# rock-slam/slam-pose_estimation

Measured on AMD Instinct MI355X. Metric: UKF predict+update filter-cycles/s, PoseWithVelocity filters, higher is better.
Workload: dtype f64

## Files before the change

slam-pose_estimation_amd/csrc/ukf_kernel16.hpp:

```cpp
#pragma once

#include <type_traits>

#include "ukf_kernel.hpp"

namespace ukfb {

template <int CTRL> UKFB_DEV float dpp_mov(float v) {
    return __builtin_bit_cast(float, __builtin_amdgcn_update_dpp(0, __builtin_bit_cast(int, v), CTRL, 0xF, 0xF, true));
}
template <int CTRL> UKFB_DEV double dpp_mov(double v) {
    const unsigned long long b = __builtin_bit_cast(unsigned long long, v);
    const int lo = __builtin_amdgcn_update_dpp(0, int(unsigned(b)), CTRL, 0xF, 0xF, true);
    const int hi = __builtin_amdgcn_update_dpp(0, int(unsigned(b >> 32)), CTRL, 0xF, 0xF, true);
    return __builtin_bit_cast(double, (unsigned long long)(unsigned)lo | ((unsigned long long)(unsigned)hi << 32));
}
template <int C> UKFB_DEV float row_bcast(float v) { return dpp_mov<0x150 + C>(v); }
template <int C> UKFB_DEV double row_bcast(double v) { return __builtin_amdgcn_update_dpp(0.0, v, 0x150 + C, 0xF, 0xF, true); }
template <int C> UKFB_DEV void fmac_bcast(float& acc, float src, float m) {
    asm volatile("v_fmac_f32_dpp %0, %1, %2 row_newbcast:%3 row_mask:0xf bank_mask:0xf" : "+v"(acc) : "v"(src), "v"(m), "n"(C));
}
template <int C> UKFB_DEV void fmac_bcast(double& acc, double src, double m) {
    asm volatile("v_fmac_f64_dpp %0, %1, %2 row_newbcast:%3 row_mask:0xf bank_mask:0xf" : "+v"(acc) : "v"(src), "v"(m), "n"(C));
}
// ... 107 lines not shown
};

constexpr float ISO_TOL_F32 = 1e-4f;
template <class T, class M> struct Layout16 {
    static constexpr int VEC = 16 / int(sizeof(T));
    static constexpr int D = M::D, S = M::S, N = 2 * D + 1, PK = D * (D + 1) / 2;
    static constexpr int LS = 14;
    static constexpr int al(int x) { return (x + VEC - 1) / VEC * VEC; }
    static constexpr int PKP = al(PK);
    static constexpr int NL = 6, ST = (D == 12) ? 6 : 7, TRIP = D + 1;
    static constexpr int LC = 0;
    static constexpr int TNL = (D * LS > N * ST) ? (D * LS - N * ST) : 0;
    static constexpr bool ORIENT64_TRIM = (M::MODEL == 1 && sizeof(T) == 8);
    static constexpr bool LAF_ROW_D = !(M::MODEL == 0 || ORIENT64_TRIM);
    static constexpr int alm(int x) { return (M::MODEL == 0 && sizeof(T) == 4) ? (x + 1) / 2 * 2 : al(x); }
    static constexpr int UEND = al(TNL + (N + 1) * ST);
    static constexpr int PKS = UEND;
    static constexpr int LAF = PKS + PKP;
    static constexpr int LAF_SZ = al((D + (LAF_ROW_D ? 1 : 0)) * ST);
    static constexpr int LAF_PAD = LAF_ROW_D ? 0 : (LAF_SZ - D * ST);
    static constexpr int MISC = LAF + LAF_SZ;
    static constexpr int MUS = MISC;
    static constexpr int ROT = MUS + alm(S);
    static constexpr int ZQ = ROT + alm(9);
    static constexpr int NSH = ZQ + 12;
    static constexpr bool SINK_IN_NSH = ORIENT64_TRIM;
    static constexpr int NSH_SINK = SINK_IN_NSH ? (NSH + 21) : (NSH + alm(21));
    static constexpr int DUM = SINK_IN_NSH ? NSH : (NSH + alm(21));
    static constexpr int PF_RAW = SINK_IN_NSH ? (NSH + alm(21)) : (DUM + alm(S));
    static_assert(!SINK_IN_NSH || (alm(21) > 21 && alm(21) >= S), "the sink fits the noise table, which has a spare slot");
    __host__ __device__ static constexpr int cv(int r, int c) { return PKS + r * (r + 1) / 2 + c; }
    static constexpr int PF = PF_RAW + (((PF_RAW * int(sizeof(T)) / 4) % 32 == 0) ? 2 * VEC : 0);
    static_assert(TNL + N * ST >= D * LS && D - NL <= ST && NL <= ST, "prediction tables");
    static_assert(PF % 2 == 0 && LS >= D && LS <= 16 && S <= 16 && D + 1 <= 16, "scratch layout");
};

template <class T, class M> constexpr int lds_bytes_per_filter16() { return Layout16<T, M>::PF * int(sizeof(T)); }

template <class T, class M, class TS = T> struct CovTab {
    using LY = Layout16<T, M>;
    static constexpr int D = M::D, NL = LY::NL, ST = LY::ST, TRIP = LY::TRIP, TR = MT<M>::TR, TC = MT<M>::TC;
    static constexpr int NAB = (D - NL) * (D - NL + 1) / 2, AEL = (NAB + 15) / 16;
    static constexpr int NRD = 8, NWR = 16, SZ = int(sizeof(T)), SZG = int(sizeof(TS));
    static constexpr int RD_PR = 0, RD_PC = 1, RD_WS = 2, RD_NZ = 4, RD_ANZ = 5;
    static constexpr int WR_TILE = 0, WR_AFF = TR * TC, WR_AFF_RD = TR * TC + AEL;
    static_assert(RD_ANZ + AEL <= NRD && WR_AFF_RD + AEL <= NWR, "covariance lane tables");
    struct Tabs {
        uint32_t rd[16][NRD];
        uint32_t wr[17][NWR];
    };
    static constexpr int tri_r(int e) {
        int r = 0;
        while ((r + 1) * (r + 2) / 2 <= e) ++r;
        return r;
    }
    static constexpr Tabs make() {
        Tabs t{};
        const uint32_t sink = uint32_t(LY::DUM * SZ);
        for (int l = 0; l < 16; ++l) {
            const int lw = (l < MT<M>::WORK_LANES) ? l : 0;
            const int R0 = int((MT<M>::TILE_R >> (4 * lw)) & 15ull), C0 = int((MT<M>::TILE_C >> (4 * lw)) & 15ull);
            const bool is_cross = R0 >= NL;
            const int half = is_cross ? 0 : (lw & 1);
            t.rd[l][RD_PR] = uint32_t((is_cross ? (LY::LAF + (R0 - NL)) : (LY::TNL + half * (TRIP * ST) + R0)) * SZ);
            t.rd[l][RD_PC] = uint32_t((LY::TNL + ((is_cross || half) ? (TRIP * ST) : 0) + C0) * SZ);
            if (SZ == 8) {
                t.rd[l][RD_WS] = 0u;
                t.rd[l][RD_WS + 1] = is_cross ? 0u : 0x3FF00000u;
            } else {
                t.rd[l][RD_WS] = is_cross ? 0u : 0x3F800000u;
            }
            const int rc0 = R0 < D ? R0 : D - 1, cc0 = C0 < D ? C0 : D - 1;
            t.rd[l][RD_NZ] = uint32_t((rc0 * D + cc0) * SZG);
            const bool writer = (l < MT<M>::WORK_LANES) && (is_cross || half == 0);
            for (int i2 = 0; i2 < TR; ++i2)
                for (int j2 = 0; j2 < TC; ++j2) {
                    const int r = R0 + i2, c = C0 + j2;
                    const bool w = writer && r < D && c <= r;
                    t.wr[l][WR_TILE + i2 * TC + j2] = w ? uint32_t(LY::cv(r, c) * SZ) : sink;
                }
            for (int k = 0; k < AEL; ++k) {
                const int e = l + 16 * k;
                const bool v = e < NAB;
                const int rr = v ? tri_r(e) : 0, cc = v ? (e - rr * (rr + 1) / 2) : 0;
                const int ar = NL + rr, ac = NL + cc;
                t.rd[l][RD_ANZ + k] = uint32_t((ar * D + ac) * SZG);
                t.wr[l][WR_AFF + k] = v ? uint32_t(LY::cv(ar, ac) * SZ) : sink;
                t.wr[l][WR_AFF_RD + k] = uint32_t(LY::cv(ar, ac) * SZ);
            }
        }
        for (int k = 0; k < NWR; ++k) t.wr[16][k] = sink;
        for (int k = 0; k < AEL; ++k) t.wr[16][WR_AFF_RD + k] = uint32_t(LY::cv(NL, NL) * SZ);
        return t;
    }
    static constexpr Tabs tabs = make();
};

template <class T, class M, class TS = T> struct OCovTab {
    using LY = Layout16<T, M>;
    static constexpr int D = M::D, NL = LY::NL, ST = LY::ST, TRIP = LY::TRIP, TR = MT<M>::TR, TC = MT<M>::TC;
    static constexpr int NAB = (D - NL) * (D - NL + 1) / 2, AEL = (NAB + 15) / 16, SZ = int(sizeof(T)), SZG = int(sizeof(TS));
    static constexpr int RD_PR = 0, RD_PC = 1, RD_FLAGS = 2, RD_NZ = 3, RD_ANZ = 4, NRD = 8;
    static constexpr int WR_TILE = 0, WR_AFF = TR * TC, WR_AFF_RD = TR * TC + AEL, NWR = 16;
    static_assert(AEL == 2 && TR * TC + 2 * AEL <= NWR && RD_ANZ + AEL <= NRD, "OrientationState lane tables");
    struct Tabs {
        uint16_t rd[16][NRD];
        uint16_t wr[17][NWR];
    };
    static constexpr int tri_r(int e) {
        int r = 0;
// ... 86 lines not shown
#endif
UKFB_DEV void keep(float& x) { asm volatile("" : "+v"(x)); }
UKFB_DEV void keep(double& x) { asm volatile("" : "+v"(x)); }

template <class T, int D, int LS, int KS = D, int PUB = KS> UKFB_DEV T chol16(T (&a)[D], T* Lc, int l, bool& ok) {
    static_assert(PUB <= KS && KS <= D, "chol16 column counts");
    bool good = true;
    const int lw = (l < D) ? l : (D - 1);
    static_for<0, KS>([&](auto kc) {
        constexpr int k = decltype(kc)::value;
        dpp_hazard_fence(a[k]);
        if constexpr (k >= PUB) {
            const T akk = row_bcast<k>(a[k]);
            good = good && (akk > T(0));
        }
        const T nt = -(a[k] * rcp_bcast<k>(a[k]));
        if constexpr (k + 1 < KS) {
            static_for<k + 1, KS>([&](auto cc) {
                constexpr int c = decltype(cc)::value;
                fmac_bcast<c>(a[c], a[k], nt);
            });
        }
    });
#pragma unroll
    for (int k = 0; k < PUB; ++k) Lc[k * LS + lw] = (l >= k) ? a[k] : T(0);
    wsync();
    const int lc = (l < PUB) ? l : (PUB - 1);
    const T pv = Lc[lc * LS + lc];
    constexpr unsigned long long NO_PIVOT = ((0xFFFFull << PUB) & 0xFFFFull) * 0x0001000100010001ull;
    ok = good && row_all(NO_PIVOT | lanes_gt(pv, T(0)));
    return fast_rsqrt(pv);
}

template <class T, int D> UKFB_DEV void load_row(const T* PKS, int l, T (&row)[D]) {
    const int lr = (l < D) ? l : (D - 1);
    const T* p = PKS + lr * (lr + 1) / 2;
#pragma unroll
    for (int j = 0; j < D; ++j) row[j] = p[j];
}

template <class T, int D, int LS> UKFB_DEV void load_column(const T* Lc, int l, T rs, T (&col)[D]) {
    const int lc = (l < D) ? l : (D - 1);
    const T w = (l < D) ? rs : T(0);
#pragma unroll
    for (int c = 0; c < D; ++c) col[c] = Lc[lc * LS + c] * w;
}

template <class T> UKFB_DEV void rot_minus(const T (&qx)[4], const T (&qy)[4], T (&r)[3]) {
    const T oc[4] = {-qy[0], -qy[1], -qy[2], qy[3]};
    T d[4];
    quat_mul(oc, qx, d);
    so3_log_fast(d, r);
}

template <class T> UKFB_DEV void rot_minus_n2(const T (&qxa)[4], const T (&qxb)[4], const T (&qy)[4], T nrm, T (&ra)[3], T (&rb)[3]) {
    const T oc[4] = {-qy[0], -qy[1], -qy[2], qy[3]};
    T da[4], db[4];
    quat_mul(oc, qxa, da);
    quat_mul(oc, qxb, db);
    if constexpr (sizeof(T) == 4) {
        so3_log_fast_n2(da, db, nrm, ra, rb);
    } else {
        so3_log_fast_n(da, nrm, ra);
        so3_log_fast_n(db, nrm, rb);
    }
}

template <class T> UKFB_DEV void rot_minus_n(const T (&qx)[4], const T (&qy)[4], T nrm, T (&r)[3]) {
    const T oc[4] = {-qy[0], -qy[1], -qy[2], qy[3]};
    T d[4];
    quat_mul(oc, qx, d);
// ... 50 lines not shown
template <class T, class M>
UKFB_DEV void sigma_pair(const T (&mu)[M::S], const T (&col)[M::D], T (&xp)[M::S], T (&xm)[M::S]) {
    constexpr int Q = MT<M>::Q, RT = MT<M>::RT, S = M::S;
#pragma unroll
    for (int s = 0; s < S; ++s) {
        if (s < Q) { xp[s] = mu[s] + col[s]; xm[s] = mu[s] - col[s]; }
        else if (s >= Q + 4) { xp[s] = mu[s] + col[s - 1]; xm[s] = mu[s] - col[s - 1]; }
    }
    const T q[4] = {mu[Q], mu[Q + 1], mu[Q + 2], mu[Q + 3]};
    const T v[3] = {col[RT], col[RT + 1], col[RT + 2]};
    T ep[4], rp[4], rm[4];
    so3_exp_fast(v, T(1), ep);
    quat_mul_pm(q, ep, rp, rm);
#pragma unroll
    for (int k = 0; k < 4; ++k) { xp[Q + k] = rp[k]; xm[Q + k] = rm[k]; }
}

template <class T, class M, class TS>
UKFB_DEV T process_noise_entry16(const TS* Rn, const TS* Racc, const T* ROT, const ProcIn<T>& pin, int r, int c) {
    constexpr int D = M::D;
    T vacc = T(0);
    if (M::MODEL == 0) {
        vacc = T(Racc[r * D + c]);
    }
    const T rn = T(Rn[r * D + c]);
    const int o = (r < 3 && c < 3) ? 0 : ((r >= 3 && r < 6 && c >= 3 && c < 6) ? 3 : -1);
    const int oo = o < 0 ? 0 : o;
    const int rr = (o < 0) ? 0 : (r - oo), cc = (o < 0) ? 0 : (c - oo);
    T acc = T(0);
#pragma unroll
    for (int m = 0; m < 3; ++m) {
        T tmp = T(0);
#pragma unroll
        for (int k = 0; k < 3; ++k) tmp += ROT[rr * 3 + k] * T(Rn[(oo + k) * D + (oo + m)]);
        acc += tmp * ROT[cc * 3 + m];
    }
    const T val = (o >= 0) ? acc : rn;
    const T scale = (M::MODEL == 0) ? pin.dt : pin.dt * pin.dt;
    const T vcv = scale * val;
    return (M::MODEL == 0 && pin.use_acc) ? vacc : vcv;
}

template <class T, class M, class TS> UKFB_DEV T plain_noise_entry16(const TS* Rn, const TS* Racc, const ProcIn<T>& pin, int r, int c) {
    constexpr int D = M::D;
    const T rn = T(Rn[r * D + c]);
    if (M::MODEL == 0) {
        const T vacc = T(Racc[r * D + c]);
        return pin.use_acc ? vacc : pin.dt * rn;
    }
    return (pin.dt * pin.dt) * rn;
}

constexpr unsigned long long tri_rows(int first) {
    unsigned long long t = 0;
    for (int i = 0; i < 16; ++i) {
        const int e = first + i;
        int r = 0;
        while ((r + 1) * (r + 2) / 2 <= e) ++r;
        t |= (unsigned long long)((e < 28 ? r : 0) & 15) << (4 * i);
    }
    return t;
}
constexpr unsigned long long tri_cols(int first) {
    unsigned long long t = 0;
    for (int i = 0; i < 16; ++i) {
        const int e = first + i;
        int r = 0;
        while ((r + 1) * (r + 2) / 2 <= e) ++r;
// ... 285 lines not shown

    bool p_commit = false, u_commit = false;

    if constexpr (DO_PREDICT) {
        if (wave_any(do_p)) {
            UKFB_MARK("p_chol");
            constexpr int NL = LY::NL, ST = LY::ST, TRIP = LY::TRIP;
            constexpr auto st_of = [](int t) constexpr { return t < MT<M>::RT ? t : t + 1; };
            T xp[S], xm[S], ref[S];
            bool ok;
            bool noise_plain = false;
            bool need_rot = false;
            T qn2 = T(1);
            {
                T mu_r[S];
#pragma unroll
                for (int s = 0; s < S; ++s) mu_r[s] = MUS[s];
                qn2 = mu_r[Q] * mu_r[Q] + mu_r[Q + 1] * mu_r[Q + 1] + mu_r[Q + 2] * mu_r[Q + 2] + mu_r[Q + 3] * mu_r[Q + 3];
                if constexpr (M::MODEL != 0)
                    noise_plain = a.noise_iso != 0 && wave_all(!do_p || m_abs(qn2 - T(1)) <= (sizeof(T) == 8 ? T(1e-9) : T(ISO_TOL_F32)));
                need_rot = !noise_plain && (M::MODEL != 0 || !wave_all(pin.use_acc));
                if (need_rot) {
                    T q[4], rot[9];
                    M::orientation(mu_r, q);
                    quat_to_matrix(q, rot);
                    T* dst = (l == 0) ? ROT : DUMP;
#pragma unroll
                    for (int k = 0; k < 9; ++k) dst[k] = rot[k];
                }
                T rs;
                {
                    T arow[D];
                    UKFB_MARK("p_chol_row");
                    load_row<T, D>(PKS, l, arow);
                    UKFB_MARK("p_chol_fact");
                    UKFB_PRIO(1);
                    rs = chol16<T, D, LS>(arow, Lc, l, ok);
                    UKFB_PRIO(0);
                    wsync();
                }
                UKFB_MARK("p_sigma");
                T col[D];
                load_column<T, D, LS>(Lc, l, rs, col);
                {
                    T* lrow = LY::LAF_ROW_D ? (LAF + ((l < D) ? l : D) * ST) : ((l < D) ? (LAF + l * ST) : DUMP);
#pragma unroll
                    for (int c = NL; c < D; ++c) lrow[c - NL] = (M::MODEL == 0) ? col[c] : col[c] * MT<M>::aff_scale(c, pin);
                    if constexpr (LY::LAF_PAD > 0) {
                        T* padp = (l == D) ? (LAF + D * ST) : DUMP;
#pragma unroll
                        for (int k = 0; k < LY::LAF_PAD; ++k) padp[k] = T(0);
                    }
                }
                sigma_pair<T, M>(mu_r, col, xp, xm);
            }
            UKFB_MARK("p_process");
            const bool pc = do_p && ok;
            sfence();
            process_fast((M*)nullptr, xp, pin);
            sfence();
            process_fast((M*)nullptr, xm, pin);
            sfence();
            UKFB_MARK("p_mean1");
#pragma unroll
            for (int s = 0; s < S; ++s)
                if (s < NL + 1) ref[s] = row_bcast<D>(xp[s]);
            const bool has_p = has_pair || has_ctr, has_m = has_pair;
// ... 161 lines not shown
                bool rebase = have_last;
                const T a2 = al[0] * al[0] + al[1] * al[1] + al[2] * al[2];
                if (rebase) {
                    const T tp = rpl[0] * rpl[0] + rpl[1] * rpl[1] + rpl[2] * rpl[2];
                    const T tm = rml[0] * rml[0] + rml[1] * rml[1] + rml[2] * rml[2];
                    rebase = wave_all(!pc || (tp <= T(2.25) && tm <= T(2.25) && a2 <= T(1e-12)));
                }
                UKFB_COUNT_VAL(2, rebase ? 1 : 0);
                if (rebase) {
                    so3_rebase_small(rpl, al, a2, rp);
                    so3_rebase_small(rml, al, a2, rm);
                } else {
                    rot_minus_n2(qp, qm, qr, qn2, rp, rm);
                }
#pragma unroll
                for (int k = 0; k < 3; ++k) {
                    rowu[RT + k] = (fu * T(0.5)) * (rp[k] + rm[k]);
                    roww[RT + k] = T(0.5) * (rp[k] - rm[k]);
                }
                T* dst = (pc && l == 0) ? MUS : DUMP;
#pragma unroll
                for (int k = 0; k < 4; ++k) dst[Q + k] = qr[k];
            }
            wsync();
            UKFB_MARK("p_cov");
            constexpr bool LANE_TABLES = (M::MODEL == 0);
            if constexpr (LANE_TABLES) {
                using CT = CovTab<T, M, TS>;
                static_assert(10 + TR <= D && 3 + TC <= NL, "Pose tile table: every tile entry is a valid (row, column)");
                constexpr int AEL = CT::AEL;
                unsigned char* const wbase = reinterpret_cast<unsigned char*>(base);
                const T* pr = reinterpret_cast<const T*>(wbase + ctr[CT::RD_PR]);
                const T* pc_ = reinterpret_cast<const T*>(wbase + ctr[CT::RD_PC]);
                uint32_t ctw[CT::NWR];
                {
                    const uint32_t* wrow = CT::tabs.wr[pc ? l : 16];
#pragma unroll
                    for (int k = 0; k < CT::WR_AFF_RD + AEL; ++k) ctw[k] = wrow[k];
                }
                const int64_t wgn = wg0_again() * a.Rn_stride;
                const TS* Rn = at(a.Rn + wgn, fc * IDX(a.Rn_stride));
                const TS* Ra = at(a.Racc + wgn, fc * IDX(a.Rn_stride));
                const auto at_off = [](const TS* p, uint32_t off, int imm) {
                    return T(reinterpret_cast<const TS*>(reinterpret_cast<const unsigned char*>(p) + off)[imm]);
                };
                const auto plain_off = [&](uint32_t off, int imm) {
                    const T rn = at_off(Rn, off, imm), vacc = at_off(Ra, off, imm);
                    return pin.use_acc ? vacc : pin.dt * rn;
                };
                const bool all_acc = wave_all(pin.use_acc);
                T acc[TR][TC], nz[TR][TC], anz[AEL];
#pragma unroll
                for (int i2 = 0; i2 < TR; ++i2)
#pragma unroll
                    for (int j2 = 0; j2 < TC; ++j2) acc[i2][j2] = nz[i2][j2] = T(0);
#pragma unroll
                for (int t = 0; t < AEL; ++t) anz[t] = T(0);
                if (all_acc) {
#pragma unroll
                    for (int i2 = 0; i2 < TR; ++i2)
#pragma unroll
                        for (int j2 = 0; j2 < TC; ++j2) nz[i2][j2] = at_off(Ra, ctr[CT::RD_NZ], i2 * D + j2);
#pragma unroll
                    for (int t = 0; t < AEL; ++t) anz[t] = at_off(Ra, ctr[CT::RD_ANZ + t], 0);
                } else {
#pragma unroll
                    for (int t = 0; t < 2; ++t) {
                        const bool v = l + G * t < NL * (NL + 1) / 2;
                        const int r = v ? int((tri_rows(G * t) >> (4 * l)) & 15ull) : 0, c = v ? int((tri_cols(G * t) >> (4 * l)) & 15ull) : 0;
                        NSH[v ? (l + G * t) : (LY::NSH_SINK - LY::NSH)] = process_noise_entry16<T, M>(Rn, Ra, ROT, pin, r, c);
                    }
                    const int lw = (l < MT<M>::WORK_LANES) ? l : 0;
                    const int R0 = int((MT<M>::TILE_R >> (4 * lw)) & 15ull), C0 = int((MT<M>::TILE_C >> (4 * lw)) & 15ull);
                    const bool is_cross = R0 >= NL;
#pragma unroll
                    for (int i2 = 0; i2 < TR; ++i2)
#pragma unroll
                        for (int j2 = 0; j2 < TC; ++j2) {
                            const int rn_ = is_cross ? 0 : (R0 + i2), cn_ = is_cross ? 0 : (C0 + j2);
                            T shaped = NSH[rn_ * (rn_ + 1) / 2 + cn_];
                            keep(shaped);
                            const T plain = plain_off(ctr[CT::RD_NZ], i2 * D + j2);
                            nz[i2][j2] = is_cross ? plain : shaped;
                        }
#pragma unroll
                    for (int t = 0; t < AEL; ++t) anz[t] = plain_off(ctr[CT::RD_ANZ + t], 0);
                }
#pragma unroll
                for (int i = 0; i < TRIP; ++i) {
                    T vr[TR], vc[TC];
#pragma unroll
                    for (int k = 0; k < TR; ++k) vr[k] = pr[i * ST + k];
#pragma unroll
                    for (int k = 0; k < TC; ++k) vc[k] = pc_[i * ST + k];
#pragma unroll
                    for (int i2 = 0; i2 < TR; ++i2)
#pragma unroll
                        for (int j2 = 0; j2 < TC; ++j2) acc[i2][j2] = fma(vr[i2], vc[j2], acc[i2][j2]);
                }
                p_commit = pc;
                st |= (do_p && !ok) ? ST_ERR_CHOLESKY : 0u;
                st |= (p_commit && !conv) ? ST_WARN_MEAN_NOCONV : 0u;
                T wsum;
                if constexpr (sizeof(T) == 8)
                    wsum = __builtin_bit_cast(T, (unsigned long long)ctr[CT::RD_WS] | ((unsigned long long)ctr[CT::RD_WS + 1] << 32));
                else
                    wsum = __builtin_bit_cast(T, ctr[CT::RD_WS]);
#pragma unroll
                for (int i2 = 0; i2 < TR; ++i2)
#pragma unroll
                    for (int j2 = 0; j2 < TC; ++j2) {
                        const T tot = fma(wsum, dpp_mov<0xB1>(acc[i2][j2]), acc[i2][j2]);
                        *reinterpret_cast<T*>(wbase + ctw[CT::WR_TILE + i2 * TC + j2]) = tot + nz[i2][j2];
                    }
#pragma unroll
                for (int t = 0; t < AEL; ++t) {
                    T old = *reinterpret_cast<const T*>(wbase + ctw[CT::WR_AFF_RD + t]);
                    keep(old);
                    *reinterpret_cast<T*>(wbase + ctw[CT::WR_AFF + t]) = old + anz[t];
                }
            } else {
                using OT = OCovTab<T, M, TS>;
                static_assert(M::MODEL == 1, "the decoded form of this phase is gone: every model has lane tables");
                constexpr int AEL = OT::AEL;
                unsigned char* const wbase = reinterpret_cast<unsigned char*>(base);
                const auto lo16 = [](uint32_t x) { return x & 0xFFFFu; };
                const auto hi16 = [](uint32_t x) { return x >> 16; };
                const T* pr = reinterpret_cast<const T*>(wbase + lo16(otr[0]));
                const T* pc_ = reinterpret_cast<const T*>(wbase + hi16(otr[0]));
                const uint32_t flags = lo16(otr[1]);
                uint32_t otw[OT::NWR / 2];
                {
                    const uint32_t* wrow = reinterpret_cast<const uint32_t*>(OT::tabs.wr[pc ? l : 16]);
#pragma unroll
                    for (int k = 0; k < (OT::WR_AFF_RD + AEL + 1) / 2; ++k) otw[k] = wrow[k];
                }
                const auto wr_off = [&](int k) { return (k & 1) ? hi16(otw[k >> 1]) : lo16(otw[k >> 1]); };
                const int64_t wgn = wg0_again() * a.Rn_stride;
// ... 27 lines not shown
#pragma unroll
                        for (int j2 = 0; j2 < TC; ++j2) acc[i2][j2] = fma(vr[i2], vc[j2], acc[i2][j2]);
                }
                p_commit = pc;
                st |= (do_p && !ok) ? ST_ERR_CHOLESKY : 0u;
                st |= (p_commit && !conv) ? ST_WARN_MEAN_NOCONV : 0u;
                {
                    const T dt2 = pin.dt * pin.dt;
                    T pl[TR][TC], apl[AEL];
#pragma unroll
                    for (int i2 = 0; i2 < TR; ++i2)
#pragma unroll
                        for (int j2 = 0; j2 < TC; ++j2) pl[i2][j2] = dt2 * rn_off(hi16(otr[1]), i2 * D + j2);
                    apl[0] = dt2 * rn_off(lo16(otr[2]), 0);
                    apl[1] = dt2 * rn_off(hi16(otr[2]), 0);
                    sfence();
                    const bool nonlin = (flags & 1u) != 0u;
                    const T wsum = nonlin ? T(1) : T(0);
                    auto store_tiles = [&](auto plain_c) {
                        constexpr bool PLAIN_NOISE = decltype(plain_c)::value;
                        int R0 = 0, C0 = 0;
                        if constexpr (!PLAIN_NOISE) {
                            const int lw = (l < MT<M>::WORK_LANES) ? l : 0;
                            R0 = int((MT<M>::TILE_R >> (4 * lw)) & 15ull);
                            C0 = int((MT<M>::TILE_C >> (4 * lw)) & 15ull);
                        }
#pragma unroll
                        for (int i2 = 0; i2 < TR; ++i2)
#pragma unroll
                            for (int j2 = 0; j2 < TC; ++j2) {
                                T nv = pl[i2][j2];
                                if constexpr (!PLAIN_NOISE) {
                                    const int rn_ = nonlin ? (R0 + i2) : 0, cn_ = nonlin ? (C0 + j2) : 0;
                                    T shaped = NSH[rn_ * (rn_ + 1) / 2 + cn_];
                                    keep(shaped);
                                    nv = nonlin ? shaped : nv;
                                }
                                const T tot = fma(wsum, dpp_mov<0xB1>(acc[i2][j2]), acc[i2][j2]);
                                *reinterpret_cast<T*>(wbase + wr_off(OT::WR_TILE + i2 * TC + j2)) = tot + nv;
                            }
                    };
                    if (noise_plain) store_tiles(std::true_type{});
                    else store_tiles(std::false_type{});
                    const T sg = MT<M>::aff_scale(NL, pin), sa = MT<M>::aff_scale(NL + 3, pin);
                    const auto scale_of = [&](int shift) {
                        const uint32_t cls = (flags >> shift) & 3u;
                        return (cls == 0u) ? sg : ((cls == 1u) ? sa : T(1));
                    };
#pragma unroll
                    for (int t = 0; t < AEL; ++t) {
                        T old = *reinterpret_cast<const T*>(wbase + wr_off(OT::WR_AFF_RD + t));
                        keep(old);
                        const T ss = scale_of(2 + 4 * t) * scale_of(4 + 4 * t);
                        *reinterpret_cast<T*>(wbase + wr_off(OT::WR_AFF + t)) = fma(ss, old, apl[t]);
                    }
                }
            }
            UKFB_MARK("p_end");
            wsync();
        }
    }

    if constexpr (DO_UPDATE) {
        if (wave_any(do_u)) {
            UKFB_MARK("u_stats");
            T zin[3];
#pragma unroll
            for (int k = 0; k < 3; ++k) zin[k] = ZQ[k];
            if (M::CHECK_MEAS_FINITE) {
                bool fin = true;
#pragma unroll
                for (int k = 0; k < 12; ++k) fin = fin && m_finite(ZQ[k]);
                st |= (do_u && !fin) ? ST_ERR_NONFINITE_MEAS : 0u;
                do_u = do_u && fin;
            }
            const int midc = M::meas_valid(mid) ? mid : (M::MODEL == 0 ? 0 : 9);
            const int m = PLAINL ? 3 : M::meas_dim(midc);
            const bool so3 = PLAINL ? false : M::meas_is_so3(midc);
            const bool need_q = so3 || (M::MODEL == 1);
            bool ok1 = true, zconv = true;
            T Sm[9], cx[3], innov[3];
            if constexpr (MULTI && sizeof(T) == 8 && M::MODEL != 0) {
#pragma unroll
                for (int k = 0; k < 9; ++k) Sm[k] = T(0);
#pragma unroll
                for (int k = 0; k < 3; ++k) cx[k] = innov[k] = T(0);
            }
            const int la = has_pair ? l : (D - 1);
            if (MT<M>::HAS_EUCLID_MEAS) {
                const int mu_id = meas_uniform_c;
                const bool uni3 = PLAINL || ((a_meas == nullptr) && (mu_id == 0 || mu_id == 4 || mu_id == 8));
                if (uni3) {
                    const int tb = (mu_id == 0) ? 0 : ((mu_id == 4) ? 6 : 9);
                    const int sb = tb + ((tb >= Q) ? 1 : 0);
#pragma unroll
                    for (int k = 0; k < 3; ++k) {
                        innov[k] = zin[k] - MUS[sb + k];
                        const int tk = tb + k;
                        const int hi = la > tk ? la : tk, lo = la > tk ? tk : la;
                        cx[k] = base[LY::cv(hi, lo)];
                    }
#pragma unroll
                    for (int r = 0; r < 3; ++r)
#pragma unroll
                        for (int c = 0; c <= r; ++c) {
                            const T sp = base[LY::cv(tb + r, tb + c)];
                            Sm[r * 3 + c] = sp + ZQ[3 + r * 3 + c];
                            if (c < r) Sm[c * 3 + r] = sp + ZQ[3 + c * 3 + r];
                        }
                } else {
                const unsigned long long sel[3] = {MT<M>::SEL0, MT<M>::SEL1, MT<M>::SEL2};
                int ti[3];
                bool used[3];
#pragma unroll
                for (int k = 0; k < 3; ++k) {
                    const int sk = int((sel[k] >> (4 * midc)) & 15ull);
                    used[k] = sk != 15;
                    const int si = used[k] ? sk : 0;
                    ti[k] = (si < Q) ? si : (si - 1);
                    T m0 = MUS[si];
                    keep(m0);
                    innov[k] = used[k] ? (zin[k] - m0) : T(0);
                    const int hi = la > ti[k] ? la : ti[k], lo = la > ti[k] ? ti[k] : la;
                    T sx = base[LY::cv(hi, lo)];
                    keep(sx);
                    cx[k] = used[k] ? sx : T(0);
                }
#pragma unroll
                for (int r = 0; r < 3; ++r)
#pragma unroll
                    for (int c = 0; c < 3; ++c) {
                        const int hi = ti[r] > ti[c] ? ti[r] : ti[c], lo = ti[r] > ti[c] ? ti[c] : ti[r];
                        const T pad = (r == c) ? T(1) : T(0);
                        T sp = base[LY::cv(hi, lo)], sq = ZQ[3 + r * 3 + c];
                        keep(sp);
                        keep(sq);
                        Sm[r * 3 + c] = (used[r] && used[c]) ? (sp + sq) : pad;
                    }
                }
            }
            if (wave_any(need_q)) {
                T zval[4] = {(0 < m) ? zin[0] : T(0), (1 < m) ? zin[1] : T(0), (2 < m) ? zin[2] : T(0), T(0)};
                if (wave_any(so3)) {
                    T qe[4];
                    so3_exp_fast(zin, T(1), qe);
#pragma unroll
                    for (int k = 0; k < 4; ++k) zval[k] = so3 ? qe[k] : zval[k];
                }
                bool okg;
                T rs;
                {
                    T arow[D];
                    load_row<T, D>(PKS, l, arow);
                    UKFB_PRIO(1);
                    rs = chol16<T, D, LS, MT<M>::ZCOLS>(arow, Lc, l, okg);
                    UKFB_PRIO(0);
                    wsync();
                }
                T zp[4], zm[4], z0[4];
                {
                    const bool zcol = l < MT<M>::ZCOLS;
                    const T w = zcol ? rs : T(0);
                    const T* colp = Lc + (zcol ? l : (MT<M>::ZCOLS - 1)) * LS;
                    const T q0[4] = {MUS[Q], MUS[Q + 1], MUS[Q + 2], MUS[Q + 3]};
                    const T cr[3] = {colp[RT] * w, colp[RT + 1] * w, colp[RT + 2] * w};
                    T e[4], qp[4], qm[4];
                    so3_exp_fast(cr, T(1), e);
                    quat_mul_pm(q0, e, qp, qm);
                    MT<M>::gen_measure(qp, qm, q0, MUS, colp, w, zp, zm, z0);
                }
                sfence();
                T zref[4] = {z0[0], z0[1], z0[2], z0[3]};
                bool zc = true;
                if (wave_any(so3 && do_u)) {
                    bool active = so3;
                    int it = 0;
                    while (wave_any(active)) {
                        T rp[3], rm[3], r0v[3], mr[3];
                        rot_minus(zp, zref, rp);
                        rot_minus(zm, zref, rm);
                        rot_minus(z0, zref, r0v);
                        T m2 = T(0);
#pragma unroll
                        for (int k = 0; k < 3; ++k) mr[k] = has_pair ? (rp[k] + rm[k]) : T(0);
                        row_allreduce_n<T, 3>(mr);
#pragma unroll
// ... 102 lines not shown
            }
            sfence();
            UKFB_MARK("u_gain");
            uint32_t asmo[4];
            {
                const uint32_t* arow = AsmTab<T, M>::tabs.off[l];
#pragma unroll
                for (int k = 0; k < 4; ++k) asmo[k] = arow[k];
            }
            T Kr[3], KSr[3];
            bool accept;
            {
                T Si[9];
                inverse3(Sm, Si);
                T maha = T(0);
#pragma unroll
                for (int r = 0; r < 3; ++r)
#pragma unroll
                    for (int c = 0; c < 3; ++c) maha += innov[r] * Si[r * 3 + c] * innov[c];
                accept = (gate_chi2_c < T(0)) || (maha <= gate_chi2_c);
#pragma unroll
                for (int c = 0; c < 3; ++c) Kr[c] = cx[0] * Si[c] + cx[1] * Si[3 + c] + cx[2] * Si[6 + c];
#pragma unroll
                for (int c = 0; c < 3; ++c) KSr[c] = Kr[0] * Sm[c] + Kr[1] * Sm[3 + c] + Kr[2] * Sm[6 + c];
            }
            const T del = Kr[0] * innov[0] + Kr[1] * innov[1] + Kr[2] * innov[2];
            sfence();
            UKFB_MARK("u_downdate_chol");
            T srow2[D], drot[3];
            bool ok2;
            T rs2;
            {
                T arow2[D];
                load_row<T, D>(PKS, l, arow2);
                const T nks[3] = {-KSr[0], -KSr[1], -KSr[2]};
                dpp_hazard_fence(Kr[0]);
                dpp_hazard_fence(Kr[1]);
                dpp_hazard_fence(Kr[2]);
                static_for<0, D>([&](auto bc) {
                    constexpr int b = decltype(bc)::value;
                    fmac_bcast<b>(arow2[b], Kr[0], nks[0]);
                    fmac_bcast<b>(arow2[b], Kr[1], nks[1]);
                    fmac_bcast<b>(arow2[b], Kr[2], nks[2]);
                    srow2[b] = arow2[b];
                    if constexpr (b >= RT && b < RT + 3) drot[b - RT] = row_bcast<b>(del);
                });
                bool short_fact = false;
                if constexpr (DO_PREDICT && PLAIN >= 1) {
                    if (a.upd_short_ok != 0) {
                        const T q00 = ZQ[3], q10 = ZQ[6], q11 = ZQ[7], q20 = ZQ[9], q21 = ZQ[10], q22 = ZQ[11];
                        const T m2 = fma(q00, q11, -(q10 * q10));
                        const T det = fma(q22, m2, fma(q20, fma(q10, q21, -(q11 * q20)), -(q21 * fma(q00, q21, -(q10 * q20)))));
                        const bool q_pd = (q00 > T(0)) && (m < 2 || m2 > T(0)) && (m < 3 || det > T(0));
                        short_fact = wave_all(!do_u || (p_commit && q_pd));
                    }
                }
                UKFB_PRIO(1);
                if (short_fact) rs2 = chol16<T, D, LS, RT + 3, RT + 3>(arow2, Lc, l, ok2);
                else rs2 = chol16<T, D, LS, D, RT + 3>(arow2, Lc, l, ok2);
                UKFB_PRIO(0);
                wsync();
            }
            sfence();
            UKFB_MARK("u_apply");
            constexpr int NC = RT + 3;
            static_assert(2 * NC <= 16, "signed rotation columns must fit one DPP row");
            T e0[4], rsg[3];
            {
                const bool plus = l < NC, minus = (l >= NC) && (l < 2 * NC);
                const int cidx = plus ? l : (minus ? (l - NC) : 0);
                const T rs_m = dpp_mov<0x110 + NC>(rs2);
                const T wc = plus ? rs2 : (minus ? -rs_m : T(0));
                T c3[3];
#pragma unroll
                for (int k = 0; k < 3; ++k) c3[k] = Lc[cidx * LS + RT + k] * wc;
                const T v0[3] = {drot[0], drot[1], drot[2]};
                const T vs[3] = {v0[0] + c3[0], v0[1] + c3[1], v0[2] + c3[2]};
                T es[4];
                so3_exp_fast(vs, T(1), es);
                static_assert(2 * NC < 16, "a lane without a signed column exists");
#pragma unroll
                for (int k = 0; k < 4; ++k) e0[k] = row_bcast<15>(es[k]);
                rot_minus_n(es, e0, T(1), rsg);
            }
            sfence();
            UKFB_MARK("u_rr_cross");
            T rr[6];
#pragma unroll
            for (int r = 0; r < 3; ++r)
#pragma unroll
                for (int c = 0; c <= r; ++c) rr[r * (r + 1) / 2 + c] = rsg[r] * rsg[c];
            row_allreduce_n<T, 6, (2 * NC <= 12) ? 3 : 4>(rr);
#pragma unroll
            for (int k = 0; k < 6; ++k) rr[k] *= T(0.5);
            T cr[3] = {T(0), T(0), T(0)};
            {
                T w[3];
#pragma unroll
                for (int k = 0; k < 3; ++k) {
                    const T rmk = dpp_mov<0x100 + NC>(rsg[k]);
                    w[k] = T(0.5) * rs2 * (rsg[k] - rmk);
                    dpp_hazard_fence(w[k]);
                }
                static_for<0, NC>([&](auto jc) {
                    constexpr int j = decltype(jc)::value;
                    const T v = Lc[j * LS + la];
                    fmac_bcast<j>(cr[0], w[0], v);
                    fmac_bcast<j>(cr[1], w[1], v);
                    fmac_bcast<j>(cr[2], w[2], v);
                });
            }
            st |= (do_u && (!ok1 || (accept && !ok2))) ? ST_ERR_CHOLESKY : 0u;
            st |= (do_u && ok1 && !accept) ? ST_REJECTED_GATE : 0u;
            st |= (do_u && ok1 && !zconv) ? ST_WARN_MEAN_NOCONV : 0u;
            u_commit = do_u && ok1 && ok2 && accept;

            sfence();
            UKFB_MARK("u_assemble");
            {
                const bool wl = u_commit && has_pair;
                unsigned char* const wbase = reinterpret_cast<unsigned char*>(base);
                constexpr uint32_t SINK = uint32_t(LY::DUM * sizeof(T));
                T* rowdst = reinterpret_cast<T*>(wbase + (wl ? asmo[0] : SINK));
#pragma unroll
                for (int b = D - 1; b >= 0; --b) {
                    rowdst[b] = srow2[b];
                    asm volatile("" ::: "memory");
                }
#pragma unroll
                for (int k = 0; k < 3; ++k) *reinterpret_cast<T*>(wbase + (wl ? asmo[1 + k] : SINK)) = cr[k];
                asm volatile("" ::: "memory");
                const bool w0 = u_commit && l == 0;
#pragma unroll
                for (int r = 0; r < 3; ++r)
#pragma unroll
                    for (int c = 0; c <= r; ++c)
                        base[w0 ? LY::cv(RT + r, RT + c) : LY::DUM] = rr[r * (r + 1) / 2 + c];
            }
            sfence();
            UKFB_MARK("u_mean");
            {
                const T q[4] = {MUS[Q], MUS[Q + 1], MUS[Q + 2], MUS[Q + 3]};
                T nq[4];
                quat_mul(q, e0, nq);
                const bool rotl = (l >= RT) && (l < RT + 3);
                const int sl = (l < RT) ? l : (l + 1);
                const bool eu = u_commit && has_pair && !rotl;
                T old = MUS[has_pair ? sl : 0];
                keep(old);
                wsync();
                MUS[eu ? sl : (LY::DUM - LY::MUS)] = old + del;
                T* dst = (u_commit && l == 0) ? (MUS + Q) : DUMP;
#pragma unroll
                for (int k = 0; k < 4; ++k) dst[k] = nq[k];
            }
            wsync();
        }
    }

    changed = changed || p_commit || u_commit;
    st_all |= st;
    if constexpr (PREFETCH) {
#pragma unroll
        for (int k = 0; k < 3; ++k) {
            pin.a[k] = nx_a[k];
            pin.w[k] = nx_w[k];
        }
        zq_l = nx_zq;
        mid_l = nx_mid;
    }
    } while (MULTI && ++cyc < ncyc);

    UKFB_MARK("commit");
    const uint32_t st = st_all;
    const int64_t wgc = wg0_again();
    TS* const cov_c = a.cov + wgc * PK;
    TS* const mu_c = a.mu + wgc * S;
    uint32_t* const status_c = a.status + wgc;
    IDX fcc = fc;
    if constexpr (!INDIRECT) asm volatile("" : "+v"(fcc));
    if (changed && fvalid) {
#pragma unroll
        for (int t = 0; t < EPL; ++t) {
            const int e = l + G * t;
            if (e < PK) *at(cov_c, fcc * PK + IDX(e)) = TS(PKS[e]);
        }
        if (l < S) *at(mu_c, fcc * S + IDX(l)) = TS(MUS[l]);
    }
    if (fvalid && l == 0) *at(status_c, fcc) = status_accumulate_c ? (*at(status_c, fcc) | st) : st;
}

}
```

Measured before the change: 899.6 million.

## Pair f64 covariance tile reads into 16-byte LDS loads, pin scalar reads

For f64 layouts with even row stride, odd-column covariance tiles are remapped so two of the three columns sit on an aligned pair. The per-row vr and two of the vc values are then fetched with one 16-byte LDS vector load each, and the remaining column uses a separate table offset. Other scalar LDS reads are routed through wavefront-scope relaxed atomic loads, likely so the compiler does not merge them into misaligned wide loads. This aims to cut LDS instruction count in the prediction covariance loop, at the cost of extra table entries, changed tile-to-column mapping and more complex lane tables.

```diff
diff --git a/slam-pose_estimation_amd/csrc/ukf_kernel16.hpp b/slam-pose_estimation_amd/csrc/ukf_kernel16.hpp
--- a/slam-pose_estimation_amd/csrc/ukf_kernel16.hpp
+++ b/slam-pose_estimation_amd/csrc/ukf_kernel16.hpp
@@ -163,6 +163,8 @@
     __host__ __device__ static constexpr int cv(int r, int c) { return PKS + r * (r + 1) / 2 + c; }
     static constexpr int PF = PF_RAW + (((PF_RAW * int(sizeof(T)) / 4) % 32 == 0) ? 2 * VEC : 0);
     static_assert(TNL + N * ST >= D * LS && D - NL <= ST && NL <= ST, "prediction tables");
+    static constexpr bool PAIR16 = (sizeof(T) == 8 && ST % 2 == 0);
+    static_assert(!PAIR16 || (TNL % 2 == 0 && LAF % 2 == 0 && PF % 2 == 0 && (TRIP * ST) % 2 == 0), "16-byte aligned table rows");
     static_assert(PF % 2 == 0 && LS >= D && LS <= 16 && S <= 16 && D + 1 <= 16, "scratch layout");
 };
 
@@ -174,6 +176,13 @@
     static constexpr int NAB = (D - NL) * (D - NL + 1) / 2, AEL = (NAB + 15) / 16;
     static constexpr int NRD = 8, NWR = 16, SZ = int(sizeof(T)), SZG = int(sizeof(TS));
     static constexpr int RD_PR = 0, RD_PC = 1, RD_WS = 2, RD_NZ = 4, RD_ANZ = 5;
+    static constexpr bool PAIRS = LY::PAIR16;
+    static constexpr int RD_PCS = 2, RD_NZS = 7;
+    static constexpr int col_of(int C0, int j2) {
+        if (!PAIRS || C0 % 2 == 0) return C0 + j2;
+        return (j2 + 1 < TC) ? (C0 + 1 + j2) : C0;
+    }
+    static_assert(!PAIRS || (TR == 2 && TC == 3 && RD_ANZ + AEL <= RD_NZS), "paired reads: 2 x 3 tiles, a spare rd slot");
     static constexpr int WR_TILE = 0, WR_AFF = TR * TC, WR_AFF_RD = TR * TC + AEL;
     static_assert(RD_ANZ + AEL <= NRD && WR_AFF_RD + AEL <= NWR, "covariance lane tables");
     struct Tabs {
@@ -194,19 +203,21 @@
             const bool is_cross = R0 >= NL;
             const int half = is_cross ? 0 : (lw & 1);
             t.rd[l][RD_PR] = uint32_t((is_cross ? (LY::LAF + (R0 - NL)) : (LY::TNL + half * (TRIP * ST) + R0)) * SZ);
-            t.rd[l][RD_PC] = uint32_t((LY::TNL + ((is_cross || half) ? (TRIP * ST) : 0) + C0) * SZ);
+            const int pcb = LY::TNL + ((is_cross || half) ? (TRIP * ST) : 0);
+            t.rd[l][RD_PC] = uint32_t((pcb + col_of(C0, 0)) * SZ);
             if (SZ == 8) {
-                t.rd[l][RD_WS] = 0u;
+                t.rd[l][RD_WS] = PAIRS ? uint32_t((pcb + col_of(C0, TC - 1)) * SZ) : 0u;
                 t.rd[l][RD_WS + 1] = is_cross ? 0u : 0x3FF00000u;
             } else {
                 t.rd[l][RD_WS] = is_cross ? 0u : 0x3F800000u;
             }
             const int rc0 = R0 < D ? R0 : D - 1, cc0 = C0 < D ? C0 : D - 1;
-            t.rd[l][RD_NZ] = uint32_t((rc0 * D + cc0) * SZG);
+            t.rd[l][RD_NZ] = uint32_t((rc0 * D + (PAIRS ? col_of(C0, 0) : cc0)) * SZG);
+            if (PAIRS) t.rd[l][RD_NZS] = uint32_t((rc0 * D + col_of(C0, TC - 1)) * SZG);
             const bool writer = (l < MT<M>::WORK_LANES) && (is_cross || half == 0);
             for (int i2 = 0; i2 < TR; ++i2)
                 for (int j2 = 0; j2 < TC; ++j2) {
-                    const int r = R0 + i2, c = C0 + j2;
+                    const int r = R0 + i2, c = col_of(C0, j2);
                     const bool w = writer && r < D && c <= r;
                     t.wr[l][WR_TILE + i2 * TC + j2] = w ? uint32_t(LY::cv(r, c) * SZ) : sink;
                 }
@@ -359,11 +370,27 @@
     return fast_rsqrt(pv);
 }
 
-template <class T, int D> UKFB_DEV void load_row(const T* PKS, int l, T (&row)[D]) {
+template <bool SINGLE, class T> UKFB_DEV T lds_rd(const T* p) {
+    if constexpr (SINGLE && sizeof(T) == 8) return __hip_atomic_load(p, __ATOMIC_RELAXED, __HIP_MEMORY_SCOPE_WAVEFRONT);
+    else return *p;
+}
+template <class T> UKFB_DEV void lds_rd_pair(const T* p, T& x0, T& x1) {
+    if constexpr (sizeof(T) == 8) {
+        typedef T pair_t __attribute__((ext_vector_type(2)));
+        const pair_t v = *static_cast<const pair_t*>(__builtin_assume_aligned(p, 16));
+        x0 = v.x;
+        x1 = v.y;
+    } else {
+        x0 = p[0];
+        x1 = p[1];
+    }
+}
+
+template <class T, int D, bool SINGLE = false> UKFB_DEV void load_row(const T* PKS, int l, T (&row)[D]) {
     const int lr = (l < D) ? l : (D - 1);
     const T* p = PKS + lr * (lr + 1) / 2;
 #pragma unroll
-    for (int j = 0; j < D; ++j) row[j] = p[j];
+    for (int j = 0; j < D; ++j) row[j] = lds_rd<SINGLE>(p + j);
 }
 
 template <class T, int D, int LS> UKFB_DEV void load_column(const T* Lc, int l, T rs, T (&col)[D]) {
@@ -480,8 +507,8 @@
     for (int m = 0; m < 3; ++m) {
         T tmp = T(0);
 #pragma unroll
-        for (int k = 0; k < 3; ++k) tmp += ROT[rr * 3 + k] * T(Rn[(oo + k) * D + (oo + m)]);
-        acc += tmp * ROT[cc * 3 + m];
+        for (int k = 0; k < 3; ++k) tmp += lds_rd<Layout16<T, M>::PAIR16>(ROT + rr * 3 + k) * T(Rn[(oo + k) * D + (oo + m)]);
+        acc += tmp * lds_rd<Layout16<T, M>::PAIR16>(ROT + cc * 3 + m);
     }
     const T val = (o >= 0) ? acc : rn;
     const T scale = (M::MODEL == 0) ? pin.dt : pin.dt * pin.dt;
@@ -833,7 +860,7 @@
                 {
                     T arow[D];
                     UKFB_MARK("p_chol_row");
-                    load_row<T, D>(PKS, l, arow);
+                    load_row<T, D, LY::PAIR16>(PKS, l, arow);
                     UKFB_MARK("p_chol_fact");
                     UKFB_PRIO(1);
                     rs = chol16<T, D, LS>(arow, Lc, l, ok);
@@ -1061,6 +1088,10 @@
                 unsigned char* const wbase = reinterpret_cast<unsigned char*>(base);
                 const T* pr = reinterpret_cast<const T*>(wbase + ctr[CT::RD_PR]);
                 const T* pc_ = reinterpret_cast<const T*>(wbase + ctr[CT::RD_PC]);
+                constexpr bool PAIRS = CT::PAIRS;
+                const T* pcs = PAIRS ? reinterpret_cast<const T*>(wbase + ctr[CT::RD_PCS]) : pc_;
+                const auto nz_off = [&](int j2) { return (PAIRS && j2 == TC - 1) ? ctr[CT::RD_NZS] : ctr[CT::RD_NZ]; };
+                const auto nz_imm = [](int j2) { return (PAIRS && j2 == TC - 1) ? 0 : j2; };
                 uint32_t ctw[CT::NWR];
                 {
                     const uint32_t* wrow = CT::tabs.wr[pc ? l : 16];
@@ -1089,7 +1120,7 @@
 #pragma unroll
                     for (int i2 = 0; i2 < TR; ++i2)
 #pragma unroll
-                        for (int j2 = 0; j2 < TC; ++j2) nz[i2][j2] = at_off(Ra, ctr[CT::RD_NZ], i2 * D + j2);
+                        for (int j2 = 0; j2 < TC; ++j2) nz[i2][j2] = at_off(Ra, nz_off(j2), i2 * D + nz_imm(j2));
 #pragma unroll
                     for (int t = 0; t < AEL; ++t) anz[t] = at_off(Ra, ctr[CT::RD_ANZ + t], 0);
                 } else {
@@ -1102,14 +1133,17 @@
                     const int lw = (l < MT<M>::WORK_LANES) ? l : 0;
                     const int R0 = int((MT<M>::TILE_R >> (4 * lw)) & 15ull), C0 = int((MT<M>::TILE_C >> (4 * lw)) & 15ull);
                     const bool is_cross = R0 >= NL;
+                    const bool odd_c = PAIRS && (C0 & 1);
+                    const int cpair = odd_c ? (C0 + 1) : C0, csingle = odd_c ? C0 : (C0 + TC - 1);
 #pragma unroll
                     for (int i2 = 0; i2 < TR; ++i2)
 #pragma unroll
                         for (int j2 = 0; j2 < TC; ++j2) {
-                            const int rn_ = is_cross ? 0 : (R0 + i2), cn_ = is_cross ? 0 : (C0 + j2);
-                            T shaped = NSH[rn_ * (rn_ + 1) / 2 + cn_];
+                            const int cj = !PAIRS ? (C0 + j2) : ((j2 == TC - 1) ? csingle : (cpair + j2));
+                            const int rn_ = is_cross ? 0 : (R0 + i2), cn_ = is_cross ? 0 : cj;
+                            T shaped = lds_rd<LY::PAIR16>(NSH + rn_ * (rn_ + 1) / 2 + cn_);
                             keep(shaped);
-                            const T plain = plain_off(ctr[CT::RD_NZ], i2 * D + j2);
+                            const T plain = plain_off(nz_off(j2), i2 * D + nz_imm(j2));
                             nz[i2][j2] = is_cross ? plain : shaped;
                         }
 #pragma unroll
@@ -1118,10 +1152,16 @@
 #pragma unroll
                 for (int i = 0; i < TRIP; ++i) {
                     T vr[TR], vc[TC];
-#pragma unroll
-                    for (int k = 0; k < TR; ++k) vr[k] = pr[i * ST + k];
-#pragma unroll
-                    for (int k = 0; k < TC; ++k) vc[k] = pc_[i * ST + k];
+                    if constexpr (PAIRS) {
+                        lds_rd_pair(pr + i * ST, vr[0], vr[1]);
+                        lds_rd_pair(pc_ + i * ST, vc[0], vc[1]);
+                        vc[2] = lds_rd<LY::PAIR16>(pcs + i * ST);
+                    } else {
+#pragma unroll
+                        for (int k = 0; k < TR; ++k) vr[k] = pr[i * ST + k];
+#pragma unroll
+                        for (int k = 0; k < TC; ++k) vc[k] = pc_[i * ST + k];
+                    }
 #pragma unroll
                     for (int i2 = 0; i2 < TR; ++i2)
 #pragma unroll
@@ -1132,7 +1172,7 @@
                 st |= (p_commit && !conv) ? ST_WARN_MEAN_NOCONV : 0u;
                 T wsum;
                 if constexpr (sizeof(T) == 8)
-                    wsum = __builtin_bit_cast(T, (unsigned long long)ctr[CT::RD_WS] | ((unsigned long long)ctr[CT::RD_WS + 1] << 32));
+                    wsum = __builtin_bit_cast(T, (unsigned long long)ctr[CT::RD_WS + 1] << 32);
                 else
                     wsum = __builtin_bit_cast(T, ctr[CT::RD_WS]);
 #pragma unroll
@@ -1226,7 +1266,7 @@
                                 T nv = pl[i2][j2];
                                 if constexpr (!PLAIN_NOISE) {
                                     const int rn_ = nonlin ? (R0 + i2) : 0, cn_ = nonlin ? (C0 + j2) : 0;
-                                    T shaped = NSH[rn_ * (rn_ + 1) / 2 + cn_];
+                                    T shaped = lds_rd<LY::PAIR16>(NSH + rn_ * (rn_ + 1) / 2 + cn_);
                                     keep(shaped);
                                     nv = nonlin ? shaped : nv;
                                 }
@@ -1289,16 +1329,16 @@
                     const int sb = tb + ((tb >= Q) ? 1 : 0);
 #pragma unroll
                     for (int k = 0; k < 3; ++k) {
-                        innov[k] = zin[k] - MUS[sb + k];
+                        innov[k] = zin[k] - lds_rd<LY::PAIR16>(MUS + sb + k);
                         const int tk = tb + k;
                         const int hi = la > tk ? la : tk, lo = la > tk ? tk : la;
-                        cx[k] = base[LY::cv(hi, lo)];
+                        cx[k] = lds_rd<LY::PAIR16>(base + LY::cv(hi, lo));
                     }
 #pragma unroll
                     for (int r = 0; r < 3; ++r)
 #pragma unroll
                         for (int c = 0; c <= r; ++c) {
-                            const T sp = base[LY::cv(tb + r, tb + c)];
+                            const T sp = lds_rd<LY::PAIR16>(base + LY::cv(tb + r, tb + c));
                             Sm[r * 3 + c] = sp + ZQ[3 + r * 3 + c];
                             if (c < r) Sm[c * 3 + r] = sp + ZQ[3 + c * 3 + r];
                         }
@@ -1345,7 +1385,7 @@
                 T rs;
                 {
                     T arow[D];
-                    load_row<T, D>(PKS, l, arow);
+                    load_row<T, D, LY::PAIR16>(PKS, l, arow);
                     UKFB_PRIO(1);
                     rs = chol16<T, D, LS, MT<M>::ZCOLS>(arow, Lc, l, okg);
                     UKFB_PRIO(0);
@@ -1514,7 +1554,7 @@
             T rs2;
             {
                 T arow2[D];
-                load_row<T, D>(PKS, l, arow2);
+                load_row<T, D, LY::PAIR16>(PKS, l, arow2);
                 const T nks[3] = {-KSr[0], -KSr[1], -KSr[2]};
                 dpp_hazard_fence(Kr[0]);
                 dpp_hazard_fence(Kr[1]);
@@ -1530,7 +1570,8 @@
                 bool short_fact = false;
                 if constexpr (DO_PREDICT && PLAIN >= 1) {
                     if (a.upd_short_ok != 0) {
-                        const T q00 = ZQ[3], q10 = ZQ[6], q11 = ZQ[7], q20 = ZQ[9], q21 = ZQ[10], q22 = ZQ[11];
+                        constexpr bool R1 = LY::PAIR16;
+                        const T q00 = lds_rd<R1>(ZQ + 3), q10 = lds_rd<R1>(ZQ + 6), q11 = lds_rd<R1>(ZQ + 7), q20 = lds_rd<R1>(ZQ + 9), q21 = lds_rd<R1>(ZQ + 10), q22 = lds_rd<R1>(ZQ + 11);
                         const T m2 = fma(q00, q11, -(q10 * q10));
                         const T det = fma(q22, m2, fma(q20, fma(q10, q21, -(q11 * q20)), -(q21 * fma(q00, q21, -(q10 * q20)))));
                         const bool q_pd = (q00 > T(0)) && (m < 2 || m2 > T(0)) && (m < 3 || det > T(0));
@@ -1555,7 +1596,7 @@
                 const T wc = plus ? rs2 : (minus ? -rs_m : T(0));
                 T c3[3];
 #pragma unroll
-                for (int k = 0; k < 3; ++k) c3[k] = Lc[cidx * LS + RT + k] * wc;
+                for (int k = 0; k < 3; ++k) c3[k] = lds_rd<LY::PAIR16>(Lc + cidx * LS + RT + k) * wc;
                 const T v0[3] = {drot[0], drot[1], drot[2]};
                 const T vs[3] = {v0[0] + c3[0], v0[1] + c3[1], v0[2] + c3[2]};
                 T es[4];
@@ -1622,7 +1663,7 @@
             sfence();
             UKFB_MARK("u_mean");
             {
-                const T q[4] = {MUS[Q], MUS[Q + 1], MUS[Q + 2], MUS[Q + 3]};
+                const T q[4] = {lds_rd<LY::PAIR16>(MUS + Q), lds_rd<LY::PAIR16>(MUS + Q + 1), lds_rd<LY::PAIR16>(MUS + Q + 2), lds_rd<LY::PAIR16>(MUS + Q + 3)};
                 T nq[4];
                 quat_mul(q, e0, nq);
                 const bool rotl = (l >= RT) && (l < RT + 3);
@@ -1665,7 +1706,7 @@
 #pragma unroll
         for (int t = 0; t < EPL; ++t) {
             const int e = l + G * t;
-            if (e < PK) *at(cov_c, fcc * PK + IDX(e)) = TS(PKS[e]);
+            if (e < PK) *at(cov_c, fcc * PK + IDX(e)) = TS(lds_rd<LY::PAIR16>(PKS + e));
         }
         if (l < S) *at(mu_c, fcc * S + IDX(l)) = TS(MUS[l]);
     }
```

Result: no change. 904.6 million (median of 6 runs) (+0.5%).
